# AliBahri94/GM3D

Measured on AMD Instinct MI355X. Metric: point-clouds/sec pretrain step (N=1024,G=64), higher is better.
Workload: dtype bf16

## Files before the change

gm3d_amd/_capi.py:

```python
import ctypes
import os

_HERE = os.path.dirname(os.path.abspath(__file__))
LIB_PATH = os.environ.get("GM3D_HIP_LIB") or os.path.join(_HERE, "lib", "libgm3d_hip.so")

GM3D_OK, GM3D_EINVAL, GM3D_EUNSUPPORTED, GM3D_ELAUNCH = 0, -1, -2, -3
GM3D_F32, GM3D_BF16 = 0, 1

_vp, _i, _f = ctypes.c_void_p, ctypes.c_int, ctypes.c_float

SIGNATURES = {
    "gm3d_abi_version": [],
    "gm3d_strerror": [_i],
    "gm3d_fps": [_vp, _i, _i, _i, _vp, _vp, _vp],
    "gm3d_gather_points": [_vp, _vp, _i, _i, _i, _i, _vp, _vp],
    "gm3d_gather_points_grad": [_vp, _vp, _i, _i, _i, _i, _vp, _vp],
    "gm3d_knn": [_vp, _vp, _i, _i, _i, _i, _vp, _vp, _vp],
    "gm3d_knn_group": [_vp, _vp, _i, _i, _i, _i, _vp, _vp, _vp, _vp],
    "gm3d_chamfer_fwd": [_vp, _vp, _i, _i, _i, _vp, _vp, _vp, _vp, _vp],
    "gm3d_chamfer_bwd": [_vp, _vp, _vp, _vp, _vp, _vp, _i, _i, _i, _vp, _vp, _vp],
    "gm3d_patch_chamfer_loss_fwd": [_vp, ctypes.c_longlong, _vp, _vp, ctypes.c_longlong, _i, _i, _i, _vp, _vp, _vp, _vp, _i, _vp],
    "gm3d_patch_chamfer_loss_bwd": [_vp, ctypes.c_longlong, _vp, _vp, ctypes.c_longlong, _vp, _vp, _vp, _i, _i, _i, _vp, _i, _vp],
    "gm3d_attention_fwd": [_vp, _vp, _vp, _i, _i, _i, _f, _i, _vp],
    "gm3d_attention_qkv_fwd": [_vp, _vp, _vp, _vp, _vp, _i, _i, _i, _i, _f, _i, _vp],
    "gm3d_attention_bwd": [_vp, _vp, _vp, _vp, _vp, _i, _i, _i, _f, _i, _vp],
    "gm3d_ln_plain_partial_rows": [_i],
    "gm3d_ln_plain_fwd": [_vp, _vp, _vp, _f, _vp, _vp, _vp, _i, _i, _i, _vp],
    "gm3d_ln_plain_bwd": [_vp, _vp, _vp, _vp, _vp, _vp, _vp, _i, _i, _i, _vp],
    "gm3d_residual_ln_fwd": [_vp, _vp, _vp, _vp, _i, _vp, _vp, _vp, _f, _vp, _vp, _vp, _vp, _i, _i, _i, _vp],
    "gm3d_residual_ln_bwd": [_vp, _vp, _vp, _vp, _vp, _vp, _vp, _i, _vp, _vp, _vp, _vp, _vp, _i, _i, _i, _vp],
    "gm3d_ln_partial_rows": [_i],
    "gm3d_colsum_finish": [_vp, _i, _i, _i, _vp, _i, _vp],
    "gm3d_colsum_finish_batched": [_vp, _i, ctypes.c_longlong, _i, _i, _i, _vp, _i, _vp],
    "gm3d_bias_gelu_fwd": [_vp, _vp, _vp, _i, _i, _i, _vp],
    "gm3d_bias_gelu_bwd": [_vp, _vp, _vp, _vp, _vp, _i, _i, _i, _vp],
    "gm3d_gelu_partial_rows": [_i],
    "gm3d_embed_partial_rows": [_i, _i, _i],
    "gm3d_moments3": [_vp, _i, _vp, _vp],
    "gm3d_pn_layer1_fwd": [_vp, _vp, _vp, _vp, _i, _i, _i, _vp],
    "gm3d_group_max_fwd": [_vp, _vp, _vp, _vp, _i, _i, _i, _i, _vp],
    "gm3d_group_max_bwd": [_vp, _vp, _vp, _i, _i, _i, _i, _vp],
    "gm3d_bn_bcast_stats": [_vp, _vp, _i, _i, _i, _vp, _i, _vp],
    "gm3d_bn_bcast_apply_relu": [_vp, _vp, _vp, _vp, _vp, _i, _i, _i, _f, _i, _vp],
    "gm3d_bn_bcast_bwd_stats": [_vp, _vp, _vp, _vp, _vp, _vp, _vp, _i, _i, _i, _vp, _f, _i, _vp],
    "gm3d_bn_bcast_bwd_apply": [_vp, _vp, _vp, _vp, _vp, _vp, _vp, _vp, _vp, _vp, _vp, _i, _i, _i, _f, _i, _vp],
    "gm3d_head_fold": [_vp, _vp, _i, _i, _vp, _vp, _vp, _i, _vp],
    "gm3d_head_rowdot": [_vp, _vp, _vp, _i, _i, _vp, _i, _vp],
    "gm3d_head_fold_bwd": [_vp, _vp, _i, _i, _i, _vp, _vp, _vp],
    "gm3d_head_outer": [_vp, _vp, _i, _i, _vp, _i, _vp],
    "gm3d_scale_translate": [_vp, _vp, _f, _f, _f, _i, _i, _vp],
    "gm3d_group_select_maps": [_vp, _i, _i, _i, _i, _vp, _vp, _vp],
    "gm3d_bn_bcast_apply_relu_sel": [_vp, _vp, _vp, _vp, _vp, _vp, _i, _i, _i, _f, _i, _vp],
    "gm3d_bn_bcast_bwd_stats_sel": [_vp, _vp, _vp, _vp, _vp, _vp, _vp, _vp, _i, _i, _i, _vp, _f, _i, _vp],
    "gm3d_bn_bcast_bwd_apply_sel": [_vp, _vp, _vp, _vp, _vp, _vp, _vp, _vp, _vp, _vp, _vp, _vp, _i, _i, _i, _f, _i, _vp],
    "gm3d_lin3_gelu_fwd": [_vp, _vp, _vp, _vp, _i, _i, _i, _vp],
    "gm3d_lin3_gelu_bwd": [_vp, _vp, _vp, _vp, _i, _i, _vp, _i, _vp],
    "gm3d_lin3_finish": [_vp, _i, _i, _vp, _vp, _vp],
    "gm3d_rank_loss": [_vp, _vp, _i, _i, _vp, _vp, _vp],
    "gm3d_rank_loss_tail": [_vp, _i, _vp, _i, _i, _vp, _vp, _vp, _vp, _vp],
    "gm3d_rank_loss_tail_bwd": [_vp, _vp, _vp, _i, _i, _i, _vp, _vp],
    "gm3d_ema_counters": [_vp, _vp, _i, _f, _f, _vp],
    "gm3d_drop_path_scales": [_vp, _vp, _i, _i, _vp, _vp],
    "gm3d_pad_cols": [_vp, ctypes.c_longlong, _i, _i, _vp, _i, _i, _vp],
    "gm3d_patch_chamfer_loss_bwd_full": [_vp, ctypes.c_longlong, _vp, _vp, ctypes.c_longlong, _vp, _vp, _vp, _i, _i, _i, _i, _vp, _i, _vp],
    "gm3d_mask_select_b": [_vp, _vp, _i, _i, _i, _i, _vp, _vp, _vp, _vp, _i, _vp],
    "gm3d_pn1_bwd_finalize": [_vp, _vp, _vp, _vp, _vp, _vp, _vp, _vp, _i, _vp],
    "gm3d_gemm_tn_bf16": [_vp, _vp, _vp, _vp, _i, _i, _i, _i, _i, _i, _vp],
    "gm3d_gemm_tn_bf16_gelu": [_vp, _vp, _vp, _vp, _vp, _i, _i, _i, _i, _i, _i, _i, _vp],
    "gm3d_gemm_tn_bf16_pool": [_vp, _vp, _vp, _vp, _vp, _vp, _i, _i, _i, _i, _i, _i, _i, _i, _vp],
    "gm3d_gemm_tn_bf16_gelu_bwd": [_vp, _vp, _vp, _vp, _vp, _vp, _i, _i, _i, _i, _i, _i, _i, _vp],
    "gm3d_gemm_tn_bf16_res": [_vp, _vp, _vp, _vp, _vp, _i, _vp, _vp, _vp, _vp, _i, _i, _i, _i, _i, _i, _vp],
    "gm3d_gemm_tn_bf16_lna": [_vp, _vp, _vp, _vp, _f, _vp, _vp, _vp, _vp, _vp, _vp, _vp, _i, _i, _i, _i, _i, _i, _i, _vp],
    "gm3d_gemm_tile_rows": [_i],
    "gm3d_gemm_tn_bf16_ring": [_vp, _vp, _vp, _vp, _i, _i, _i, _i, _i, _i, _i, _vp],
    "gm3d_gemm_tn_bf16_ws": [_vp, _vp, _vp, _vp, _i, _i, _i, _i, _i, _i, _vp],
    "gm3d_gemm_tn_bf16_ws_pool": [_vp, _vp, _vp, _vp, _vp, _vp, _i, _i, _i, _i, _i, _i, _i, _i, _vp],
    "gm3d_gemm_ws_supported": [_i, _i, _i],
    "gm3d_gemm_tn_bf16_ws_poolg": [_vp, _vp, _vp, _vp, _vp, _vp, _i, _i, _i, _i, _i, _i, _i, _i, _i, _vp],
# ... 104 lines not shown
```

gm3d_amd/csrc/attention.hip:

```cpp
#include "mfma.hpp"

namespace gm3d {

constexpr int HD = 64;
constexpr int VLD = 72;

__device__ __forceinline__ int permk(int s, int j, int hh) { return 16 * s + 8 * (j >> 2) + 4 * hh + (j & 3); }

__device__ __forceinline__ bf16x8 ld8(const bf16_t* p) { return *reinterpret_cast<const bf16x8*>(p); }
__device__ __forceinline__ bf16x8 ld8_perm(const bf16_t* row, int k0, int s, int hh) {
    const bf16x4 a = *reinterpret_cast<const bf16x4*>(row + k0 + 16 * s + 4 * hh);
    const bf16x4 b = *reinterpret_cast<const bf16x4*>(row + k0 + 16 * s + 8 + 4 * hh);
    bf16x8 v;
#pragma unroll
    for (int j = 0; j < 4; ++j) { v[j] = a[j]; v[4 + j] = b[j]; }
    return v;
}
__device__ __forceinline__ bf16x8 ld8_col_perm(const bf16_t* M, int ld, int k0, int s, int hh, int col) {
    bf16x8 v;
#pragma unroll
    for (int j = 0; j < 8; ++j) v[j] = M[(size_t)(k0 + permk(s, j, hh)) * ld + col];
    return v;
}

// ... 266 lines not shown
    const int qrow = 32 * qb + r;
    for (int s = 0; s < 32; ++s) {
        const int d = 2 * s + hh;
        const float bq = Qs[rot(qrow, d)];
#pragma unroll
        for (int t = 0; t < MT; ++t)
            if (t < NK) st[t] = MFMA_F32(Ks[rot(32 * t + r, d)], bq, st[t]);
    }
    float m = -INFINITY;
#pragma unroll
    for (int t = 0; t < MT; ++t)
#pragma unroll
        for (int g = 0; g < 16; ++g) {
            const int key = 32 * t + crow(g, hh);
            st[t][g] = key < T ? st[t][g] * scale : -INFINITY;
            m = fmaxf(m, st[t][g]);
        }
    m = fmaxf(m, __shfl_xor(m, 32));
    float sum = 0.f;
#pragma unroll
    for (int t = 0; t < MT; ++t)
#pragma unroll
        for (int g = 0; g < 16; ++g) {
            st[t][g] = expf(st[t][g] - m);
            sum += st[t][g];
        }
    sum += __shfl_xor(sum, 32);
    const float inv = 1.0f / sum;

    f32x16 o0 = zero16(), o1 = zero16();
#pragma unroll
    for (int s = 0; s < 16; ++s) {
        const int key = crow(s, hh);
#pragma unroll
        for (int t = 0; t < MT; ++t)
            if (t < NK) {
                const float p = st[t][s] * inv;
                o0 = MFMA_F32(p, Vs[rot(32 * t + key, r)], o0);
                o1 = MFMA_F32(p, Vs[rot(32 * t + key, 32 + r)], o1);
            }
    }
    float* og = out + (size_t)b * T * H * HD + (size_t)h * HD;
#pragma unroll
    for (int g = 0; g < 16; ++g) {
        const int q = 32 * qb + crow(g, hh);
        if (q < T) {
            og[(size_t)q * H * HD + r] = o0[g];
            og[(size_t)q * H * HD + 32 + r] = o1[g];
        }
    }
    if (lse && hh == 0 && qrow < T) lse[((size_t)b * H + h) * T + qrow] = m + logf(sum);
}

template <int NT>
__global__ __launch_bounds__(128 * NT) void attn_bwd_bf16_kernel(const bf16_t* __restrict__ qkv, const bf16_t* __restrict__ out,
                                                                const bf16_t* __restrict__ dout, const float* __restrict__ lse,
                                                                bf16_t* __restrict__ dqkv, int T, int H, float scale) {
    extern __shared__ __attribute__((aligned(16))) unsigned char smem[];
    constexpr int ROWS = 32 * NT, IMG = ROWS * 128;
    unsigned char* Qi = smem;
    unsigned char* Ki = Qi + IMG;
    unsigned char* Vi = Ki + IMG;
    unsigned char* Di = Vi + IMG;
    float* Ls = reinterpret_cast<float*>(Di + IMG);
    float* Del = Ls + ROWS;
    const int b = blockIdx.x / H, h = blockIdx.x % H;
    const int tid = threadIdx.x, lane = tid & 63, w = __builtin_amdgcn_readfirstlane(tid >> 6);
    const int r = lane & 31, hh = lane >> 5;
    const size_t rs = (size_t)3 * H * HD, os = (size_t)H * HD;
    const bf16_t* Qg = qkv + (size_t)b * T * rs + (size_t)h * HD;
    const bf16_t* Og = out + (size_t)b * T * os + (size_t)h * HD;
    const bf16_t* Dg = dout + (size_t)b * T * os + (size_t)h * HD;
    {
        uint4 v[6], d[2], o[2];
#pragma unroll
        for (int i = 0; i < 6; ++i) {
            const int c = tid + i * 128 * NT;
            const int tile = c / (ROWS * 8), rc = c - tile * (ROWS * 8), row = rc >> 3, ch = rc & 7;
            const int rr = row < T ? row : T - 1;
            v[i] = *reinterpret_cast<const uint4*>(Qg + (size_t)rr * rs + (size_t)tile * os + ch * 8);
        }
#pragma unroll
        for (int i = 0; i < 2; ++i) {
            const int c = tid + i * 128 * NT, row = c >> 3, ch = c & 7;
            const int rr = row < T ? row : T - 1;
            d[i] = *reinterpret_cast<const uint4*>(Dg + (size_t)rr * os + ch * 8);
            o[i] = *reinterpret_cast<const uint4*>(Og + (size_t)rr * os + ch * 8);
        }
#pragma unroll
        for (int i = 0; i < 6; ++i) {
            const int c = tid + i * 128 * NT;
            const int tile = c / (ROWS * 8), rc = c - tile * (ROWS * 8), row = rc >> 3, ch = rc & 7;
            *reinterpret_cast<uint4*>(smem + tile * IMG + img_off(row, ch)) = row < T ? v[i] : make_uint4(0, 0, 0, 0);
        }
#pragma unroll
        for (int i = 0; i < 2; ++i) {
            const int c = tid + i * 128 * NT, row = c >> 3, ch = c & 7;
            const uint4 dz = row < T ? d[i] : make_uint4(0, 0, 0, 0);
            *reinterpret_cast<uint4*>(Di + img_off(row, ch)) = dz;
            const bf16x8 d8 = *reinterpret_cast<const bf16x8*>(&dz), o8 = *reinterpret_cast<const bf16x8*>(&o[i]);
            float acc = 0.f;
#pragma unroll
            for (int j = 0; j < 8; ++j) acc += (float)o8[j] * (float)d8[j];
            acc += __shfl_xor(acc, 1);
            acc += __shfl_xor(acc, 2);
            acc += __shfl_xor(acc, 4);
            if (ch == 0) {
                Del[row] = acc;
                Ls[row] = row < T ? lse[((size_t)b * H + h) * T + row] : 0.f;
            }
        }
    }
    __syncthreads();

    bf16_t* dQg = dqkv + (size_t)b * T * rs + (size_t)h * HD;
    const int cb = 16 * ((lane >> 4) & 1);
    f32x16 x0 = zero16(), x1 = zero16(), y0 = zero16(), y1 = zero16();
    if (w < NT) {
        const int kt = w;
        const int key = 32 * kt + r;
        for (int qt = 0; qt < NT; ++qt) {
            f32x16 s = zero16(), dp = zero16();
#pragma unroll
            for (int ks = 0; ks < 4; ++ks) {
                const int ch = 2 * ks + hh;
                s = mfma_bf16(img_row(Qi, 32 * qt + r, ch), img_row(Ki, key, ch), s);
                dp = mfma_bf16(img_row(Di, 32 * qt + r, ch), img_row(Vi, key, ch), dp);
            }
#pragma unroll
            for (int g = 0; g < 16; ++g) {
                const int q = 32 * qt + crow(g, hh);
                const float p = (q < T && key < T) ? __expf(s[g] * scale - Ls[q]) : 0.f;
                s[g] = p;
                dp[g] = p * (dp[g] - Del[q]);
            }
#pragma unroll
            for (int ks = 0; ks < 2; ++ks) {
                const bf16x8 pa = cvt8(s, ks, 1.0f);
                const bf16x8 da = cvt8(dp, ks, scale);
                x0 = mfma_bf16(img_tr8(Di, 32 * qt, ks, hh, cb, lane), pa, x0);
                x1 = mfma_bf16(img_tr8(Di, 32 * qt, ks, hh, 32 + cb, lane), pa, x1);
                y0 = mfma_bf16(img_tr8(Qi, 32 * qt, ks, hh, cb, lane), da, y0);
                y1 = mfma_bf16(img_tr8(Qi, 32 * qt, ks, hh, 32 + cb, lane), da, y1);
            }
        }
    }
    else {
        const int qt = w - NT;
        const int q = 32 * qt + r;
        const float lq = Ls[q], dq_ = Del[q];
        for (int kt = 0; kt < NT; ++kt) {
            f32x16 s = zero16(), dp = zero16();
// ... 148 lines not shown
    if (dtype != GM3D_F32 && dtype != GM3D_BF16) return GM3D_EINVAL;
    if ((long long)B * H > 0x7fffffffLL) return GM3D_EUNSUPPORTED;
    return GM3D_OK;
}

}

extern "C" int gm3d_attention_fwd(const void* qkv, void* out, float* lse, int B, int T, int H, float scale,
                                  int dtype, gm3d_stream_t stream) {
    using namespace gm3d;
    int rc = attn_check(qkv, out, B, T, H, dtype);
    if (rc != GM3D_OK) return rc;
    if (B == 0) return GM3D_OK;
    const int nt = (T + 31) / 32;
    if (dtype == GM3D_BF16) {
        const size_t lds = (size_t)3 * 32 * nt * 128;
#define GM3D_AF(NT_) launch_lds<attn_fwd_bf16_kernel<NT_>>(dim3(B * H), dim3(64 * NT_), lds, stream, (const bf16_t*)qkv, (bf16_t*)out, lse, T, H, scale)
        return nt == 1 ? GM3D_AF(1) : nt == 2 ? GM3D_AF(2) : nt == 3 ? GM3D_AF(3) : GM3D_AF(4);
#undef GM3D_AF
    }
    const int threads = 64 * nt;
    const int rows = T <= 64 ? 64 : 128;
    const size_t lds = sizeof(float) * 3 * rows * 64;
    return T <= 64 ? launch_lds<attn_fwd_f32_kernel<2>>(dim3(B * H), dim3(threads), lds, stream, (const float*)qkv, (float*)out, lse, T, H, scale)
                   : launch_lds<attn_fwd_f32_kernel<4>>(dim3(B * H), dim3(threads), lds, stream, (const float*)qkv, (float*)out, lse, T, H, scale);
}

extern "C" int gm3d_attention_qkv_fwd(const void* h, const void* wqkv, void* out, float* lse, void* qkv_out, int B, int T, int H,
                                      int C, float scale, int dtype, gm3d_stream_t stream) {
    using namespace gm3d;
    if (!h || !wqkv || !out || B < 0 || T < 1 || H < 1) return GM3D_EINVAL;
    if (dtype != GM3D_BF16 || T > 64 || C != QA_C || H * HD != C) return GM3D_EUNSUPPORTED;
    if ((((size_t)h | (size_t)wqkv | (size_t)out | (size_t)qkv_out) & 15)) return GM3D_EUNSUPPORTED;
    if ((long long)B * H > 0x7ffffff0LL) return GM3D_EUNSUPPORTED;
    if (B == 0) return GM3D_OK;
    constexpr int LOOK = 1;
    const size_t lds = (size_t)(LOOK + 1) * QA_STAGE;
    const int total = B * H, grid = (total + 7) / 8 * 8;
    return qkv_out ? launch_lds<attn_qkv_fwd_bf16_kernel<LOOK, true>>(dim3(grid), dim3(256), lds, stream, (const bf16_t*)h, (const bf16_t*)wqkv,
                                 (bf16_t*)out, lse, (bf16_t*)qkv_out, T, H, scale, total)
                   : launch_lds<attn_qkv_fwd_bf16_kernel<LOOK, false>>(dim3(grid), dim3(256), lds, stream, (const bf16_t*)h, (const bf16_t*)wqkv,
                                 (bf16_t*)out, lse, (bf16_t*)nullptr, T, H, scale, total);
}

extern "C" int gm3d_attention_bwd(const void* qkv, const void* out, const void* dout, const float* lse, void* dqkv,
                                  int B, int T, int H, float scale, int dtype, gm3d_stream_t stream) {
    using namespace gm3d;
    int rc = attn_check(qkv, out, B, T, H, dtype);
    if (rc != GM3D_OK) return rc;
    if (!dout || !lse || !dqkv) return GM3D_EINVAL;
    if (B == 0) return GM3D_OK;
    const int nt = (T + 31) / 32;
    if (dtype == GM3D_BF16) {
        const size_t lds = (size_t)4 * 32 * nt * 128 + 2 * 32 * nt * sizeof(float);
#define GM3D_AB(NT_)                                                                                                      \
    launch_lds<attn_bwd_bf16_kernel<NT_>>(dim3(B * H), dim3(128 * NT_), lds, stream, (const bf16_t*)qkv, (const bf16_t*)out, (const bf16_t*)dout, lse, \
                (bf16_t*)dqkv, T, H, scale)
        return nt == 1 ? GM3D_AB(1) : nt == 2 ? GM3D_AB(2) : nt == 3 ? GM3D_AB(3) : GM3D_AB(4);
#undef GM3D_AB
    }
    const int threads = 128 * nt;
    const int rows = T <= 64 ? 64 : 128;
    const size_t lds = sizeof(float) * (4 * rows * 64 + 2 * rows);
    return T <= 64 ? launch_lds<attn_bwd_f32_kernel<2>>(dim3(B * H), dim3(threads), lds, stream, (const float*)qkv, (const float*)out,
                                 (const float*)dout, lse, (float*)dqkv, T, H, scale)
                   : launch_lds<attn_bwd_f32_kernel<4>>(dim3(B * H), dim3(threads), lds, stream, (const float*)qkv, (const float*)out,
                                 (const float*)dout, lse, (float*)dqkv, T, H, scale);
}
```

gm3d_amd/fused.py:

```python
import weakref

import contextlib

import torch

from ._capi import lib
from . import gemm
from . import streams as _streams
from .ops import _launch, _ptr, _stream, _DT

LNC = 384


class _WeightCache:

    def __init__(self):
        self._c = {}
        self._pinned = {}
        self._groups = []

    def pin(self, model, dtype=torch.bfloat16, static=False):
        src = [p for p in model.parameters() if p.dim() >= 2 and p.dtype == torch.float32 and p.is_cuda
               and not self._is_pinned(p)]
        if not src:
            return
        dst = [torch.empty_like(p, dtype=dtype) for p in src]
        for p, d in zip(src, dst):
            self._pinned[p.data_ptr()] = (d, weakref.ref(p))
        if static:
            with torch.no_grad():
                torch._foreach_copy_(dst, [p.detach() for p in src])
            return
        self._groups.append(([p.detach() for p in src], dst))
        with torch.no_grad():
            torch._foreach_copy_(dst, self._groups[-1][0])

    def pin_view(self, p, shadow):
        self._pinned[p.data_ptr()] = (shadow, weakref.ref(p))
        gemm.forget_transposes()

    def _is_pinned(self, p):
        hit = self._pinned.get(p.data_ptr())
        return hit is not None and hit[1]() is p

    def refresh(self):
        with torch.no_grad():
            for src, dst in self._groups:
                torch._foreach_copy_(dst, src)

    def get(self, w, dtype):
        if w.dtype == dtype:
            return w
        hit = self._pinned.get(w.data_ptr())
        if hit is not None and hit[1]() is w and hit[0].dtype == dtype:
            return hit[0]
# ... 173 lines not shown


DEFER_HEAD_WGRAD = False


def _run_deferred(reg, own=()):
    jobs, reg["deferred"] = reg["deferred"], []
    cur = torch.cuda.current_stream()
    reqs = []
    for tensors, rq in jobs:
        for t in tensors:
            t.record_stream(cur)
        reqs += rq
    res = _wgrad_many(reqs + list(own)) if (reqs or own) else []
    return res[len(reqs):]

_wgrad_streams = {}
ASYNC_WGRAD = True


class async_wgrad:

    def __init__(self, device, min_blocks=None, defer_heads=False):
        self.dev, self.min_blocks = torch.device(device), (WGRAD_MIN_BLOCKS if min_blocks is None else min_blocks)
        self.defer_heads = bool(defer_heads)

    def __enter__(self):
        if ASYNC_WGRAD and self.dev.type == "cuda":
            key = (self.dev.type, self.dev.index)
            if key not in _wgrad_streams:
                _wgrad_streams[key] = torch.cuda.Stream(device=self.dev)
            _ASYNC_WGRAD.update(stream=_wgrad_streams[key], used=False, min_blocks=self.min_blocks, defer_heads=self.defer_heads)
            if self.defer_heads:
                gemm.prepare_transposes()
        return self

    def __exit__(self, *exc):
        reg = _ASYNC_WGRAD
        ws, used = reg["stream"], reg["used"]
        if reg.get("defer_heads"):
            gemm.drop_transposes()
        reg.update(stream=None, used=False, defer_heads=False)
        if reg["deferred"]:
            if exc[0] is None:
                _run_deferred(reg)
            reg["deferred"] = []
        if ws is not None and used:
            _streams.join(ws)
        return False


DIRECT_INPUT_GRADS = True
FUSE_QKV_ATTENTION = True
PER_BLOCK = 11


def block_params(block):
    return [block.norm1.weight, block.norm1.bias, block.attn.qkv.weight, block.attn.proj.weight, block.attn.proj.bias,
            block.norm2.weight, block.norm2.bias, block.mlp.fc1.weight, block.mlp.fc1.bias, block.mlp.fc2.weight,
            block.mlp.fc2.bias]


class TransformerStackFn(torch.autograd.Function):

    @staticmethod
    def forward(ctx, x, pos, meta, final_w, final_b, *params):
        with torch.autocast("cuda", enabled=False):
            return TransformerStackFn._forward(ctx, x, pos, meta, final_w, final_b, *params)

    @staticmethod
    def _forward(ctx, x, pos, meta, final_w, final_b, *params):
        g = TransformerStackFn._forward_gen(ctx, x, pos, meta, final_w, final_b, *params)
        while True:
            try:
                next(g)
            except StopIteration as done:
                return done.value

    @staticmethod
    def _forward_gen(ctx, x, pos, meta, final_w, final_b, *params):
        B, T, C = x.shape
        assert C == LNC and len(params) % PER_BLOCK == 0
        nblk = len(params) // PER_BLOCK
        adt, H, scale, eps = meta["adt"], meta["num_heads"], meta["scale"], meta["eps"]
        R = B * T
        posa = pos.reshape(R, C).to(adt).contiguous()
        need = meta["grad"] and any(ctx.needs_input_grad)
        y = bias = rs = None
        if x.dtype == adt and adt != torch.float32:
            res, y = None, x.reshape(R, C).contiguous()
        else:
            res = x.reshape(R, C).float().contiguous()
        saved = []
        dev = x.device
        if need:
            H1 = torch.empty(nblk, R, C, dtype=adt, device=dev)
            A = torch.empty(nblk, R, C, dtype=adt, device=dev)
            H2 = torch.empty(nblk, R, C, dtype=adt, device=dev)
            GG = torch.empty(nblk, R, 4 * C, dtype=adt, device=dev)
        fuse_ln = (gemm.ENABLED and gemm.FUSE_LN and gemm.FUSE_GELU and adt == torch.bfloat16 and x.is_cuda
                   and all(gemm.supported(posa, weight_cache.get(params[i * PER_BLOCK + k], adt)) or k == 9
                           for i in range(nblk) for k in (2, 3, 7)))
        st1 = None
        for i in range(nblk):
            ln1w, ln1b, wqkv, wproj, bproj, ln2w, ln2b, w1, b1, w2, b2 = params[i * PER_BLOCK:(i + 1) * PER_BLOCK]
            dp1, dp2 = meta["dp"][i]
# ... 69 lines not shown
            return TransformerStackFn._backward(ctx, dout)

    @staticmethod
    def _backward(ctx, dout):
        meta, (B, T, C), nblk = ctx.meta, ctx.shape, ctx.nblk
        adt, H, scale = meta["adt"], meta["num_heads"], meta["scale"]
        R = B * T
        tens = ctx.saved_tensors
        final_w, xf, mf, rf, H1, A, H2, GG = tens[:8]
        params = tens[8:8 + nblk * PER_BLOCK]
        saved = tens[8 + nblk * PER_BLOCK:]
        grads = [None] * (nblk * PER_BLOCK)
        dev = dout.device
        dh = dout.reshape(R, C).to(adt).contiguous()
        DO = torch.empty(nblk, R, C, dtype=adt, device=dev)
        DF = torch.empty(nblk, R, 4 * C, dtype=adt, device=dev)
        DP = torch.empty(nblk, R, C, dtype=adt, device=dev)
        DQ = torch.empty(nblk, R, 3 * C, dtype=adt, device=dev)
        PLN = torch.empty(2 * nblk + 1, lib.gm3d_ln_partial_rows(R), 3 * C, dtype=torch.float32, device=dev)
        SLN = torch.empty(2 * nblk + 1, 3, C, dtype=torch.float32, device=dev)
        w2s = [weight_cache.get(params[i * PER_BLOCK + 9], adt) for i in range(nblk)]
        fuse_mlp_bwd = gemm.ENABLED and gemm.FUSE_GELU_BWD and adt == torch.bfloat16 and dh.is_cuda
        if fuse_mlp_bwd:
            W2T, WPT, W1T, WQT = gemm.stacked_transposes(
                [w2s] + [[weight_cache.get(params[i * PER_BLOCK + k], adt) for i in range(nblk)] for k in (3, 7, 2)])
        dma_bwd = fuse_mlp_bwd and gemm.dma_supported(dh.reshape(R, C), W2T[0])
        bm_bwd = gemm.dma_bm(R)
        PGL = torch.empty(nblk, ((R + bm_bwd - 1) // bm_bwd if dma_bwd else gemm.tile_rows(R)) if fuse_mlp_bwd
                          else lib.gm3d_gelu_partial_rows(R), 4 * C, dtype=torch.float32, device=dev)
        SGL = torch.empty(nblk, 4 * C, dtype=torch.float32, device=dev)
        dp2_last = meta["dp"][nblk - 1][1]
        G, d_o, _ = residual_ln_bwd(dh, None, xf, mf, rf, final_w, dp2_last, T, None, True, adt, R, dy=DO[nblk - 1],
                                    partial=PLN[2 * nblk])
        g_final_w, g_final_b, db2 = SLN[2 * nblk, 0], SLN[2 * nblk, 1], SLN[2 * nblk, 2]
        dpos = torch.zeros(R, C, dtype=torch.float32, device=dev) if nblk == 1 else None
        for i in range(nblk - 1, -1, -1):
            ln1w, ln1b, wqkv, wproj, bproj, ln2w, ln2b, w1, b1, w2, b2 = params[i * PER_BLOCK:(i + 1) * PER_BLOCK]
            u, m1, r1, qkv, lse, x1, m2, r2, f = saved[i * 9:(i + 1) * 9]
            dp1 = meta["dp"][i][0]
            dp2_prev = meta["dp"][i - 1][1] if i > 0 else None
            gi = grads[i * PER_BLOCK:(i + 1) * PER_BLOCK]
            gi[10] = db2
            if fuse_mlp_bwd:
                df = (gemm.linear_gelu_bwd_dma(d_o, W2T[i], f, b1, DF[i], PGL[i], bm=bm_bwd) if dma_bwd
                      else gemm.linear_gelu_bwd(d_o, W2T[i], f, b1, DF[i], PGL[i]))
            else:
                dg = gemm.mm_nn(d_o, weight_cache.get(w2, adt))
                df, _ = bias_gelu_bwd(dg, f, b1, adt, df=DF[i], partial=PGL[i])
            gi[8] = SGL[i]
            dh2 = gemm.mm(df, W1T[i]) if fuse_mlp_bwd else gemm.mm_nn(df, weight_cache.get(w1, adt))
            dx1, d_p, _ = residual_ln_bwd(dh2, G, x1, m2, r2, ln2w, dp1, T, None, True, adt, R, dy=DP[i],
                                          partial=PLN[2 * i + 1])
            gi[5], gi[6], gi[4] = SLN[2 * i + 1, 0], SLN[2 * i + 1, 1], SLN[2 * i + 1, 2]
            da = gemm.mm(d_p, WPT[i]) if fuse_mlp_bwd else gemm.mm_nn(d_p, weight_cache.get(wproj, adt))
            dqkv = _attention_bwd(qkv, A[i], da, lse, B, T, H, scale, dqkv=DQ[i])
            dh1 = gemm.mm(dqkv, WQT[i]) if fuse_mlp_bwd else gemm.mm_nn(dqkv, weight_cache.get(wqkv, adt))
            last = DIRECT_INPUT_GRADS and i == 0 and nblk > 1 and adt != torch.float32 and ctx.in_dtypes == (adt, adt)
            if last:
                dx_a = torch.empty(R, C, dtype=adt, device=dev)
                dpos_a = torch.empty(R, C, dtype=adt, device=dev)
                G, _, _ = residual_ln_bwd(dh1, dx1, u, m1, r1, ln1w, None, T, dpos, True, adt, R, dy=dx_a, partial=PLN[0],
                                          acc_out=dpos_a)
            else:
                G, d_o, _ = residual_ln_bwd(dh1, dx1, u, m1, r1, ln1w, dp2_prev, T, dpos, i > 0, adt, R,
                                            dy=DO[i - 1] if i > 0 else None, partial=PLN[2 * i])
            if dpos is None:
                dpos = G
            gi[0], gi[1] = SLN[2 * i, 0], SLN[2 * i, 1]
            db2 = SLN[2 * i, 2]
            grads[i * PER_BLOCK:(i + 1) * PER_BLOCK] = gi
        finish_batched(PLN, SLN.view(2 * nblk + 1, 3 * C))
        finish_batched(PGL, SGL)
        from .optim import grad_slots
        def slot(k):
            ps = [params[i * PER_BLOCK + k] for i in range(nblk)]
            return grad_slots.stacked(ps) if dev.type == "cuda" and all(p.grad is None for p in ps) else None
        reg = _ASYNC_WGRAD
        fresh = dev.type == "cuda" and all(params[i * PER_BLOCK + k].grad is None for i in range(nblk) for k in (9, 7, 3, 2))
        ws = reg["stream"] if fresh else None
        slots = [slot(k) for k in (9, 7, 3, 2)] if fresh else [None] * 4
        jobs = [(DO, GG), (DF, H2), (DP, A), (DQ, H1)]
        own = [(dy_, x_, sl) for (dy_, x_), sl in zip(jobs, slots)]
        if ws is not None and nblk < reg["min_blocks"] and all(sl is not None for sl in slots):
            reg["deferred"].append(((DO, GG, DF, H2, DP, A, DQ, H1), own))
            gw2, gw1, gwp, gwq = slots
        else:
            if ws is not None and nblk >= reg["min_blocks"]:
                _streams.fork(ws, who="fused.TransformerStackFn.backward: weight-gradient stream (async_wgrad region)")
                reg["used"] = True
                for t in (DO, GG, DF, H2, DP, A, DQ, H1):
                    t.record_stream(ws)
            else:
                ws = None
            with (torch.cuda.stream(ws) if ws is not None else contextlib.nullcontext()):
                gw2, gw1, gwp, gwq = _run_deferred(reg, own) if ws is not None else _wgrad_many(own)
        for i in range(nblk):
            grads[i * PER_BLOCK + 9], grads[i * PER_BLOCK + 7] = gw2[i], gw1[i]
            grads[i * PER_BLOCK + 3], grads[i * PER_BLOCK + 2] = gwp[i], gwq[i]
        if last:
            return (dx_a.view(B, T, C), dpos_a.view(B, T, C), None, g_final_w, g_final_b) + tuple(grads)
        dx = G.view(B, T, C).to(ctx.in_dtypes[0])
        return (dx, dpos.view(B, T, C).to(ctx.in_dtypes[1]), None, g_final_w, g_final_b) + tuple(grads)


def run_stack(blocks, final_norm, x, pos, training):
    from . import models_mae_learn_loss as M
    blocks = list(blocks)
    adt = torch.bfloat16 if (torch.is_autocast_enabled() and torch.get_autocast_dtype("cuda") == torch.bfloat16) \
# ... 5 lines not shown
        probs += [p, p]
    scales = M.drop_path_scales(B, probs, training, x.device)
    dp = [(scales[2 * i], scales[2 * i + 1]) for i in range(len(blocks))]
    meta = {"num_heads": blocks[0].attn.num_heads, "scale": blocks[0].attn.scale, "eps": blocks[0].norm1.eps,
            "final_eps": final_norm.eps, "adt": adt, "dp": dp, "grad": torch.is_grad_enabled()}
    params = []
    for b in blocks:
        params += block_params(b)
    ns = NOGRAD_SPLIT
    if (ns > 1 and x.is_cuda and not training and B % ns == 0 and B // ns >= 16
            and not (torch.is_grad_enabled() and (x.requires_grad or params[0].requires_grad))):
        main = torch.cuda.current_stream()
        h = B // ns
        x, pos = x.contiguous(), pos.contiguous()
        outs = [None] * ns
        streams = [main] + [_split_stream(x.device, j) for j in range(1, ns)]
        for side in streams[1:]:
            _streams.fork(side, main, who="fused.run_stack: parallel inference chain (NOGRAD_SPLIT)")
            x.record_stream(side)
            pos.record_stream(side)
        if LOCKSTEP:
            T_, C_ = x.shape[1], x.shape[2]
            out = torch.empty(B, T_, C_, dtype=adt, device=x.device)
            for side in streams[1:]:
                out.record_stream(side)
            with torch.autocast("cuda", enabled=False), torch.no_grad():
                gens = [TransformerStackFn._forward_gen(_NoCtx(), x[j * h:(j + 1) * h], pos[j * h:(j + 1) * h],
                                                        dict(meta, hout=out[j * h:(j + 1) * h].view(h * T_, C_)), final_norm.weight,
                                                        final_norm.bias, *params) for j in range(ns)]
                live = ns
                while live:
                    for j in range(ns):
                        if gens[j] is None:
                            continue
                        with torch.cuda.stream(streams[j]):
                            try:
                                next(gens[j])
                            except StopIteration as done:
                                outs[j], gens[j] = done.value, None
                                live -= 1
        else:
            for j in range(1, ns):
                with torch.cuda.stream(streams[j]):
                    outs[j] = TransformerStackFn.apply(x[j * h:(j + 1) * h], pos[j * h:(j + 1) * h], meta, final_norm.weight,
                                                       final_norm.bias, *params)
            outs[0] = TransformerStackFn.apply(x[:h], pos[:h], meta, final_norm.weight, final_norm.bias, *params)
        for j in range(1, ns):
            _streams.join(streams[j], main)
            outs[j].record_stream(main)
        return out if LOCKSTEP else torch.cat(outs, dim=0)
    return TransformerStackFn.apply(x, pos, meta, final_norm.weight, final_norm.bias, *params)


class _NoCtx:
    needs_input_grad = ()

    def save_for_backward(self, *a):
        pass


LOCKSTEP = True
NOGRAD_SPLIT = 2
_split_streams = {}


def _split_stream(device, j=1):
    key = (device.type, device.index, j)
    if key not in _split_streams:
        _split_streams[key] = torch.cuda.Stream(device=device)
    return _split_streams[key]
```

include/gm3d.h:

```cpp
#ifndef GM3D_H
#define GM3D_H
#include <stdint.h>

#ifdef __cplusplus
extern "C" {
#endif

typedef void *gm3d_stream_t;

enum {
    GM3D_OK = 0,
    GM3D_EINVAL = -1,
    GM3D_EUNSUPPORTED = -2,
    GM3D_ELAUNCH = -3
};

enum { GM3D_F32 = 0, GM3D_BF16 = 1 };

int gm3d_abi_version(void);
const char *gm3d_strerror(int code);

int gm3d_fps(const float *xyz, int B, int N, int npoint, int32_t *idx, float *centers,
             gm3d_stream_t stream);

int gm3d_gather_points(const float *feat, const int32_t *idx, int B, int C, int N, int M,
                       float *out, gm3d_stream_t stream);

int gm3d_gather_points_grad(const float *grad_out, const int32_t *idx, int B, int C, int N, int M,
                            float *grad_feat, gm3d_stream_t stream);

int gm3d_knn(const float *ref, const float *query, int B, int N, int G, int k,
             float *dist, int64_t *idx, gm3d_stream_t stream);

int gm3d_knn_group(const float *xyz, const float *center, int B, int N, int G, int k,
                   int64_t *idx, float *neighborhood, float *neighborhood_org,
                   gm3d_stream_t stream);

int gm3d_chamfer_fwd(const float *xyz1, const float *xyz2, int P, int n, int m,
                     float *dist1, float *dist2, int32_t *idx1, int32_t *idx2,
                     gm3d_stream_t stream);

int gm3d_chamfer_bwd(const float *xyz1, const float *xyz2, const int32_t *idx1, const int32_t *idx2,
                     const float *grad_dist1, const float *grad_dist2, int P, int n, int m,
                     float *gxyz1, float *gxyz2, gm3d_stream_t stream);

int gm3d_attention_fwd(const void *qkv, void *out, float *lse, int B, int T, int H,
                       float scale, int dtype, gm3d_stream_t stream);

int gm3d_attention_qkv_fwd(const void *h, const void *wqkv, void *out, float *lse, void *qkv_out,
                           int B, int T, int H, int C, float scale, int dtype, gm3d_stream_t stream);

int gm3d_attention_bwd(const void *qkv, const void *out, const void *dout, const float *lse,
                       void *dqkv, int B, int T, int H, float scale, int dtype,
                       gm3d_stream_t stream);

int gm3d_patch_chamfer_loss_fwd(const void *pred, long long pred_bstride, const float *target, const long long *ids,
                                long long ids_bstride, int B, int T, int M, float *matrix, int32_t *idx1, int32_t *idx2,
                                float *mean_out, int dtype, gm3d_stream_t stream);
int gm3d_patch_chamfer_loss_bwd(const void *pred, long long pred_bstride, const float *target, const long long *ids,
                                long long ids_bstride, const int32_t *idx1, const int32_t *idx2, const float *gmean, int B, int T,
                                int M, void *dpred, int dtype, gm3d_stream_t stream);
int gm3d_patch_chamfer_loss_bwd_full(const void *pred, long long pred_bstride, const float *target, const long long *ids,
                                     long long ids_bstride, const int32_t *idx1, const int32_t *idx2, const float *gmean, int B, int T,
                                     int M, int lead, void *dpred, int dtype, gm3d_stream_t stream);
int gm3d_patch_chamfer_l1_loss_fwd(const void *pred, long long pred_bstride, const float *target, const long long *ids,
                                   long long ids_bstride, int B, int T, int M, float *matrix, int32_t *idx1, int32_t *idx2,
                                   float *mean_out, int dtype, gm3d_stream_t stream);
int gm3d_patch_chamfer_l1_loss_bwd(const void *pred, long long pred_bstride, const float *target, const long long *ids,
                                   long long ids_bstride, const int32_t *idx1, const int32_t *idx2, const float *gmean, int B, int T,
                                   int M, void *dpred, int dtype, gm3d_stream_t stream);

int gm3d_ln_plain_partial_rows(int R);
int gm3d_ln_plain_fwd(const void *x, const float *gamma, const float *beta, float eps, void *h, float *mean, float *rstd, int R,
                      int C, int dtype, gm3d_stream_t stream);
int gm3d_ln_plain_bwd(const void *dh, const void *x, const float *mean, const float *rstd, const float *gamma, void *dx,
                      float *partial, int R, int C, int dtype, gm3d_stream_t stream);
int gm3d_add_ln_fwd(const void *x, const void *y, const float *ybias, const float *rowscale, int rows_per_sample, const void *z,
                    const float *gamma, const float *beta, float eps, void *s_out, void *h, float *mean, float *rstd, int R, int C,
                    int dtype, gm3d_stream_t stream);
int gm3d_add_ln_bwd(const void *dh, const void *gin, const void *x, const float *mean, const float *rstd, const float *gamma,
                    const float *rowscale, int rows_per_sample, void *dx, void *dy, float *partial, int nsum, int R, int C, int dtype,
                    gm3d_stream_t stream);
int gm3d_add_ln_bwd_acc(const void *dh, const void *gin, const void *x, const float *mean, const float *rstd, const float *gamma,
                        const float *rowscale, int rows_per_sample, void *dx, void *dy, float *partial, int nsum, void *acc,
                        int acc_mode, int R, int C, int dtype, gm3d_stream_t stream);


int gm3d_residual_ln_fwd(const float *res, const void *y, const float *bias, const float *rowscale,
                         int rows_per_sample, const void *add, const float *gamma, const float *beta,
                         float eps, float *out_res, void *h, float *mean, float *rstd, int R, int C,
                         int dtype, gm3d_stream_t stream);

int gm3d_residual_ln_bwd(const void *dh, const float *gin, const float *x, const float *mean,
                         const float *rstd, const float *gamma, const float *rowscale, int rows_per_sample,
                         float *dx, void *dy, float *acc, void *acc_out, float *partial, int R, int C, int dtype,
                         gm3d_stream_t stream);
int gm3d_ln_partial_rows(int R);

int gm3d_colsum_finish(const float *partial, int nrows, int pitch, int ncols, float *out, int accumulate,
                       gm3d_stream_t stream);

int gm3d_colsum_finish_batched(const float *partial, int njobs, long long job_stride, int nrows, int pitch, int ncols,
                               float *out, int out_stride, gm3d_stream_t stream);

int gm3d_bias_gelu_fwd(const void *f, const float *bias, void *g, int R, int C, int dtype,
                       gm3d_stream_t stream);
int gm3d_bias_gelu_bwd(const void *dg, const void *f, const float *bias, void *df, float *partial, int R,
// ... 267 lines not shown
```

Baseline: 17100.

## Fuse output-projection backward GEMM into attention backward kernel

Adds a PROJ variant of the bf16 attention backward kernel that computes dout = dy @ Wproj^T for its own (batch, head) slice. It does this with an MFMA GEMM fed by a triple-buffered global-to-LDS ring, and writes the result straight into the LDS image that the attention backward already uses. The aim is to drop the separate projection GEMM launch and the round trip of the da tensor through global memory. In exchange each block recomputes its head's 64-column slice from the full 384-wide dy row, needs more LDS for the ring, and the path is only taken when C=384, T<=64 and inputs are bf16.

```diff
diff --git a/gm3d_amd/_capi.py b/gm3d_amd/_capi.py
--- a/gm3d_amd/_capi.py
+++ b/gm3d_amd/_capi.py
@@ -24,6 +24,7 @@
     "gm3d_attention_fwd": [_vp, _vp, _vp, _i, _i, _i, _f, _i, _vp],
     "gm3d_attention_qkv_fwd": [_vp, _vp, _vp, _vp, _vp, _i, _i, _i, _i, _f, _i, _vp],
     "gm3d_attention_bwd": [_vp, _vp, _vp, _vp, _vp, _i, _i, _i, _f, _i, _vp],
+    "gm3d_attention_proj_bwd": [_vp, _vp, _vp, _vp, _vp, _vp, _i, _i, _i, _i, _f, _i, _vp],
     "gm3d_ln_plain_partial_rows": [_i],
     "gm3d_ln_plain_fwd": [_vp, _vp, _vp, _f, _vp, _vp, _vp, _i, _i, _i, _vp],
     "gm3d_ln_plain_bwd": [_vp, _vp, _vp, _vp, _vp, _vp, _vp, _i, _i, _i, _vp],
diff --git a/gm3d_amd/csrc/attention.hip b/gm3d_amd/csrc/attention.hip
--- a/gm3d_amd/csrc/attention.hip
+++ b/gm3d_amd/csrc/attention.hip
@@ -342,10 +342,17 @@
     if (lse && hh == 0 && qrow < T) lse[((size_t)b * H + h) * T + qrow] = m + logf(sum);
 }
 
-template <int NT>
+constexpr int PB_LOOK = 2, PB_NBUF = PB_LOOK + 1;
+constexpr size_t attn_bwd_lds(int nt, bool proj) {
+    const size_t images = (size_t)4 * 32 * nt * 128 + 2 * 32 * nt * sizeof(float), ring = (size_t)PB_NBUF * (32 * nt + 64) * 128;
+    return proj && ring > images ? ring : images;
+}
+
+template <int NT, bool PROJ = false>
 __global__ __launch_bounds__(128 * NT) void attn_bwd_bf16_kernel(const bf16_t* __restrict__ qkv, const bf16_t* __restrict__ out,
                                                                 const bf16_t* __restrict__ dout, const float* __restrict__ lse,
-                                                                bf16_t* __restrict__ dqkv, int T, int H, float scale) {
+                                                                bf16_t* __restrict__ dqkv, int T, int H, float scale,
+                                                                const bf16_t* __restrict__ wt, int total) {
     extern __shared__ __attribute__((aligned(16))) unsigned char smem[];
     constexpr int ROWS = 32 * NT, IMG = ROWS * 128;
     unsigned char* Qi = smem;
@@ -354,7 +361,14 @@
     unsigned char* Di = Vi + IMG;
     float* Ls = reinterpret_cast<float*>(Di + IMG);
     float* Del = Ls + ROWS;
-    const int b = blockIdx.x / H, h = blockIdx.x % H;
+    int b, h;
+    if constexpr (PROJ) {
+        const int logical = xcd_tile(blockIdx.x, gridDim.x);
+        if (logical >= total) return;
+        b = logical / H, h = logical - b * H;
+    } else {
+        b = blockIdx.x / H, h = blockIdx.x % H;
+    }
     const int tid = threadIdx.x, lane = tid & 63, w = __builtin_amdgcn_readfirstlane(tid >> 6);
     const int r = lane & 31, hh = lane >> 5;
     const size_t rs = (size_t)3 * H * HD, os = (size_t)H * HD;
@@ -374,8 +388,59 @@
         for (int i = 0; i < 2; ++i) {
             const int c = tid + i * 128 * NT, row = c >> 3, ch = c & 7;
             const int rr = row < T ? row : T - 1;
-            d[i] = *reinterpret_cast<const uint4*>(Dg + (size_t)rr * os + ch * 8);
+            if (!PROJ) d[i] = *reinterpret_cast<const uint4*>(Dg + (size_t)rr * os + ch * 8);
             o[i] = *reinterpret_cast<const uint4*>(Og + (size_t)rr * os + ch * 8);
+        }
+        if constexpr (PROJ) {
+            constexpr int NW = 2 * NT, STAGE = (ROWS + 64) * 128, PA = ROWS / 8, PIECES = (PA + 8) / NW;
+            static_assert(PIECES * NW == PA + 8 && QA_KT > PB_LOOK, "whole pieces per wave; the prologue fills PB_LOOK stages");
+            const unsigned lds0 = lds_addr(smem);
+            const int prow = lane >> 3, pslot = lane & 7;
+            const bf16_t* src[PIECES];
+#pragma unroll
+            for (int i = 0; i < PIECES; ++i) {
+                const int p = w + NW * i;
+                if (p < PA) {
+                    const int row = 8 * p + prow;
+                    const int t = row < T ? row : T - 1;
+                    src[i] = dout + ((size_t)b * T + t) * QA_C + ((pslot ^ swz(row)) << 3);
+                } else {
+                    const int row = 8 * (p - PA) + prow;
+                    src[i] = wt + ((size_t)h * HD + row) * QA_C + ((pslot ^ swz(row)) << 3);
+                }
+            }
+#define GM3D_PB_STAGE(ST)                                                                                \
+    {                                                                                                    \
+        const unsigned base = lds0 + ((ST) % PB_NBUF) * STAGE;                                           \
+        _Pragma("unroll") for (int i = 0; i < PIECES; ++i) glds16(src[i] + (ST) * 64, base + 1024 * (w + NW * i)); \
+    }
+            f32x16 acc = zero16();
+            const int wm = (w >> 1) * 32, wn = (w & 1) * 32;
+#pragma unroll
+            for (int s = 0; s < PB_LOOK; ++s) GM3D_PB_STAGE(s)
+#define GM3D_PB_ITER(KT_)                                                                                                   \
+    {                                                                                                                       \
+        asm volatile("s_waitcnt vmcnt(%0) lgkmcnt(0)" ::"n"(PIECES * ((QA_KT - 1 - (KT_)) < (PB_LOOK - 1) ? (QA_KT - 1 - (KT_)) : (PB_LOOK - 1))) : "memory"); \
+        __builtin_amdgcn_s_barrier();                                                                                       \
+        if ((KT_) + PB_LOOK < QA_KT) GM3D_PB_STAGE((KT_) + PB_LOOK)                                                         \
+        const unsigned char* as = smem + ((KT_) % PB_NBUF) * STAGE;                                                         \
+        const unsigned char* ws = as + ROWS * 128;                                                                          \
+        _Pragma("unroll") for (int s = 0; s < 4; ++s)                                                                       \
+            acc = mfma_bf16(img_row(ws, wn + r, 2 * s + hh), img_row(as, wm + r, 2 * s + hh), acc);                         \
+    }
+            GM3D_PB_ITER(0) GM3D_PB_ITER(1) GM3D_PB_ITER(2) GM3D_PB_ITER(3) GM3D_PB_ITER(4) GM3D_PB_ITER(5)
+#undef GM3D_PB_ITER
+#undef GM3D_PB_STAGE
+            static_assert(QA_KT == 6, "GM3D_PB_ITER is written out for six K-stages");
+            __syncthreads();
+            const int token = wm + r;
+#pragma unroll
+            for (int q = 0; q < 4; ++q) {
+                bf16x4 pk;
+#pragma unroll
+                for (int e = 0; e < 4; ++e) pk[e] = token < T ? (bf16_t)acc[4 * q + e] : (bf16_t)0.0f;
+                *reinterpret_cast<bf16x4*>(Di + img_off(token, (wn >> 3) + q) + 8 * hh) = pk;
+            }
         }
 #pragma unroll
         for (int i = 0; i < 6; ++i) {
@@ -383,11 +448,19 @@
             const int tile = c / (ROWS * 8), rc = c - tile * (ROWS * 8), row = rc >> 3, ch = rc & 7;
             *reinterpret_cast<uint4*>(smem + tile * IMG + img_off(row, ch)) = row < T ? v[i] : make_uint4(0, 0, 0, 0);
         }
+        if constexpr (PROJ) {
+            __syncthreads();
+#pragma unroll
+            for (int i = 0; i < 2; ++i) {
+                const int c = tid + i * 128 * NT, row = c >> 3, ch = c & 7;
+                d[i] = *reinterpret_cast<const uint4*>(Di + img_off(row, ch));
+            }
+        }
 #pragma unroll
         for (int i = 0; i < 2; ++i) {
             const int c = tid + i * 128 * NT, row = c >> 3, ch = c & 7;
             const uint4 dz = row < T ? d[i] : make_uint4(0, 0, 0, 0);
-            *reinterpret_cast<uint4*>(Di + img_off(row, ch)) = dz;
+            if (!PROJ) *reinterpret_cast<uint4*>(Di + img_off(row, ch)) = dz;
             const bf16x8 d8 = *reinterpret_cast<const bf16x8*>(&dz), o8 = *reinterpret_cast<const bf16x8*>(&o[i]);
             float acc = 0.f;
 #pragma unroll
@@ -642,10 +715,10 @@
     if (B == 0) return GM3D_OK;
     const int nt = (T + 31) / 32;
     if (dtype == GM3D_BF16) {
-        const size_t lds = (size_t)4 * 32 * nt * 128 + 2 * 32 * nt * sizeof(float);
+        const size_t lds = attn_bwd_lds(nt, false);
 #define GM3D_AB(NT_)                                                                                                      \
-    launch_lds<attn_bwd_bf16_kernel<NT_>>(dim3(B * H), dim3(128 * NT_), lds, stream, (const bf16_t*)qkv, (const bf16_t*)out, (const bf16_t*)dout, lse, \
-                (bf16_t*)dqkv, T, H, scale)
+    launch_lds<attn_bwd_bf16_kernel<NT_>>(dim3(B * H), dim3(128 * NT_), lds, stream, (const bf16_t*)qkv, (const bf16_t*)out, (const bf16_t*)dout, \
+                lse, (bf16_t*)dqkv, T, H, scale, (const bf16_t*)nullptr, B * H)
         return nt == 1 ? GM3D_AB(1) : nt == 2 ? GM3D_AB(2) : nt == 3 ? GM3D_AB(3) : GM3D_AB(4);
 #undef GM3D_AB
     }
@@ -657,3 +730,20 @@
                    : launch_lds<attn_bwd_f32_kernel<4>>(dim3(B * H), dim3(threads), lds, stream, (const float*)qkv, (const float*)out,
                                  (const float*)dout, lse, (float*)dqkv, T, H, scale);
 }
+
+extern "C" int gm3d_attention_proj_bwd(const void* qkv, const void* out, const void* dy, const void* wt, const float* lse, void* dqkv,
+                                       int B, int T, int H, int C, float scale, int dtype, gm3d_stream_t stream) {
+    using namespace gm3d;
+    if (B < 0 || T < 1 || H < 1 || (dtype != GM3D_F32 && dtype != GM3D_BF16)) return GM3D_EINVAL;
+    if (dtype != GM3D_BF16 || T > 64 || C != QA_C || (long long)H * HD != C) return GM3D_EUNSUPPORTED;
+    if ((((size_t)qkv | (size_t)out | (size_t)dy | (size_t)wt | (size_t)dqkv) & 15)) return GM3D_EUNSUPPORTED;
+    if ((long long)B * H > 0x7ffffff0LL) return GM3D_EUNSUPPORTED;
+    if (B == 0) return GM3D_OK;
+    if (!qkv || !out || !dy || !wt || !lse || !dqkv) return GM3D_EINVAL;
+    const int total = B * H, grid = (total + 7) / 8 * 8;
+#define GM3D_APB(NT_)                                                                                                                \
+    launch_lds<attn_bwd_bf16_kernel<NT_, true>>(dim3(grid), dim3(128 * NT_), attn_bwd_lds(NT_, true), stream, (const bf16_t*)qkv, (const bf16_t*)out, \
+                                                (const bf16_t*)dy, lse, (bf16_t*)dqkv, T, H, scale, (const bf16_t*)wt, total)
+    return T <= 32 ? GM3D_APB(1) : GM3D_APB(2);
+#undef GM3D_APB
+}
diff --git a/gm3d_amd/fused.py b/gm3d_amd/fused.py
--- a/gm3d_amd/fused.py
+++ b/gm3d_amd/fused.py
@@ -1,6 +1,5 @@
+import contextlib
 import weakref
-
-import contextlib
 
 import torch
 
@@ -280,6 +279,7 @@
 
 DIRECT_INPUT_GRADS = True
 FUSE_QKV_ATTENTION = True
+FUSE_PROJ_ATTENTION_BWD = True
 PER_BLOCK = 11
 
 
@@ -455,8 +455,11 @@
             dx1, d_p, _ = residual_ln_bwd(dh2, G, x1, m2, r2, ln2w, dp1, T, None, True, adt, R, dy=DP[i],
                                           partial=PLN[2 * i + 1])
             gi[5], gi[6], gi[4] = SLN[2 * i + 1, 0], SLN[2 * i + 1, 1], SLN[2 * i + 1, 2]
-            da = gemm.mm(d_p, WPT[i]) if fuse_mlp_bwd else gemm.mm_nn(d_p, weight_cache.get(wproj, adt))
-            dqkv = _attention_bwd(qkv, A[i], da, lse, B, T, H, scale, dqkv=DQ[i])
+            if FUSE_PROJ_ATTENTION_BWD and fuse_mlp_bwd and attention_proj_bwd_supported(qkv, A[i], d_p, WPT[i], DQ[i], T, H):
+                dqkv = _attention_proj_bwd(qkv, A[i], d_p, WPT[i], lse, B, T, H, scale, DQ[i])
+            else:
+                da = gemm.mm(d_p, WPT[i]) if fuse_mlp_bwd else gemm.mm_nn(d_p, weight_cache.get(wproj, adt))
+                dqkv = _attention_bwd(qkv, A[i], da, lse, B, T, H, scale, dqkv=DQ[i])
             dh1 = gemm.mm(dqkv, WQT[i]) if fuse_mlp_bwd else gemm.mm_nn(dqkv, weight_cache.get(wqkv, adt))
             last = DIRECT_INPUT_GRADS and i == 0 and nblk > 1 and adt != torch.float32 and ctx.in_dtypes == (adt, adt)
             if last:
@@ -568,6 +571,19 @@
     return TransformerStackFn.apply(x, pos, meta, final_norm.weight, final_norm.bias, *params)
 
 
+def _attention_proj_bwd(qkv, out, dy, wt, lse, B, T, H, scale, dqkv):
+    C = dy.shape[1]
+    _launch("gm3d_attention_proj_bwd", {"B": B, "T": T, "H": H, "C": C, "dtype": str(qkv.dtype)}, lib.gm3d_attention_proj_bwd, _ptr(qkv),
+            _ptr(out), _ptr(dy), _ptr(wt), _ptr(lse), _ptr(dqkv), B, T, H, C, float(scale), _DT[qkv.dtype], _stream())
+    return dqkv
+
+
+def attention_proj_bwd_supported(qkv, out, dy, wt, dqkv, T, H):
+    return (dy.is_cuda and all(t.dtype == torch.bfloat16 and t.is_contiguous() and t.data_ptr() % 16 == 0 for t in (qkv, out, dy, wt, dqkv))
+            and T <= 64 and dy.shape[1] == 384 == H * 64 and tuple(wt.shape) == (384, 384) and qkv.shape[1] == 1152 == dqkv.shape[1]
+            and out.shape[1] == 384)
+
+
 class _NoCtx:
     needs_input_grad = ()
 
diff --git a/include/gm3d.h b/include/gm3d.h
--- a/include/gm3d.h
+++ b/include/gm3d.h
@@ -53,6 +53,9 @@
 int gm3d_attention_bwd(const void *qkv, const void *out, const void *dout, const float *lse,
                        void *dqkv, int B, int T, int H, float scale, int dtype,
                        gm3d_stream_t stream);
+
+int gm3d_attention_proj_bwd(const void *qkv, const void *out, const void *dy, const void *wt, const float *lse,
+                            void *dqkv, int B, int T, int H, int C, float scale, int dtype, gm3d_stream_t stream);
 
 int gm3d_patch_chamfer_loss_fwd(const void *pred, long long pred_bstride, const float *target, const long long *ids,
                                 long long ids_bstride, int B, int T, int M, float *matrix, int32_t *idx1, int32_t *idx2,
```

Measured after the change: 17220 (median of 6 runs). About the same (+0.7%).
